# USTC-Computer-Vision/tracking

Hardware: AMD Instinct MI355X
Metric: MixtureOfGaussianV2BGS throughput (Mpixels/s; concurrent 1080p30 streams in streams_1080p30) (higher is better)
Workload: dtype f32

## Files before the change

### tracking_amd/csrc/bgs_hip.hip

```cpp
#include "../../include/bgs_hip.h"

#include <hip/hip_runtime.h>

#include <algorithm>
#include <chrono>
#include <cmath>
#include <cstdarg>
#include <cstdio>
#include <cstdlib>
#include <cstring>
#include <mutex>
#include <new>
#include <string>
#include <atomic>
#include <vector>

#include "kernel_gmg.h"
#include "kernel_ingest.h"
#include "kernel_kde.h"
#include "kernel_dp2.h"
#include "kernel_lb.h"
#include "kernel_cc.h"
#include "kernel_dp.h"
#include "kernel_mog1.h"
// ... 294 lines not shown
  static const bool debug = getenv("BGS_DEBUG_STAT") != nullptr;
  if (debug)
    fprintf(stderr, "[bgs] mog2 auto: %u record slots sampled, %.3f live, %.3f needed after the summaries -> mode %d (now %d)\n", total, lf, nf, want, e->mog2_sparse_now);
  if (want != e->mog2_sparse_now && (clear || want == e->mog2_sparse_want)) e->mog2_sparse_now = want;
  e->mog2_sparse_want = want;
}
void mog2_stat_post(bgs_engine* e, hipStream_t s) {
  const int i = (int)(e->stat_seq % bgs_engine::kStatSlots);
  (void)hipMemcpyAsync(e->h_stat + 3 * i, e->d_stat, 3 * sizeof(unsigned), hipMemcpyDeviceToHost, s);
  (void)hipMemsetAsync(e->d_stat, 0, 3 * sizeof(unsigned), s);
  (void)hipEventRecord(e->stat_ev[i], s);
  e->stat_posted[i] = true;
  e->stat_seq++;
}

int launch_mog2(bgs_engine* e, bgs::Mog2Args& a, hipStream_t s, bool timed = true) {
  const bgs_params& p = e->p;
  a.shadow = p.mog2_detect_shadows && (!p.enable_threshold || ((p.mog2_shadow_value > p.threshold) != (255 > p.threshold)));
  a.want_bg = a.bgimg != nullptr, a.packed = a.fg_bits != nullptr;
  a.xcd_swizzle = e->xcd_swizzle, a.complete = e->mog2_complete;
  const bool autom = timed && e->mog2_sparse == 3;
  if (autom) mog2_stat_read(e);
  int mode = e->mog2_sparse == 3 ? e->mog2_sparse_now : e->mog2_sparse;
  if (mode >= 4 && (a.shadow || a.want_bg)) mode = 2;
  if (autom && mode != 4) {
    const unsigned n = e->mog2_launches++;
    if ((n & (n < 64 ? 3u : 15u)) == 0) mode = 4;
  }
  a.sparse = mode;
  a.stat = (autom && mode == 4) ? e->d_stat : nullptr;
  if (a.packed && a.npix % 64) return fail(BGS_ERR_UNSUPPORTED, "packed mask needs pixels %% 64 == 0");
  Timed t(e, s, "mog2_update_kernel", timed);
  const dim3 grid(blocks_for(a.npix)), block(bgs::kBlock);
  unsigned every = 1;
  while (grid.x / every > 256) every <<= 1;
  a.stat_mask = every - 1;
  static const unsigned lds_pad = getenv("BGS_MOG2_LDS_PAD") ? (unsigned)std::max(0, std::min(65536, atoi(getenv("BGS_MOG2_LDS_PAD")))) : 0u;
  if (mode >= 4)
    hipLaunchKernelGGL((bgs::mog2_update_kernel<bgs::kMog2Filter>), grid, block, lds_pad, s, a);
  else if (mode >= 2)
    hipLaunchKernelGGL((bgs::mog2_update_kernel<bgs::kMog2Count>), grid, block, lds_pad, s, a);
  else
    hipLaunchKernelGGL((bgs::mog2_update_kernel<bgs::kMog2Eager>), grid, block, lds_pad, s, a);
  if (a.stat) mog2_stat_post(e, s);
  return BGS_OK;
}

void mog1_fill_args(const bgs_engine* e, bgs::Mog1Args& m, double lr) {
  const bgs_params& p = e->p;
  const int C = e->ch;
  const double defaultNoiseSigma = 30 * 0.5;
  m.alpha = (float)lr, m.T = (float)p.mog1_background_ratio, m.vT = (float)p.mog1_var_threshold;
  m.w0 = (float)0.05;
  m.sk0 = C == 3 ? (float)(m.w0 / (defaultNoiseSigma * 2 * std::sqrt(3.))) : (float)(m.w0 / (defaultNoiseSigma * 2));
  m.var0 = (float)(defaultNoiseSigma * defaultNoiseSigma * 4);
  m.minVar = (float)(p.mog1_noise_sigma * p.mog1_noise_sigma);
  m.thr = p.threshold, m.enable_thr = p.enable_threshold, m.packed = m.fg_bits != nullptr, m.xcd_swizzle = e->xcd_swizzle;
}

void mog2_fill_args(const bgs_engine* e, bgs::Mog2Args& m, double lr) {
  const bgs_params& p = e->p;
  m.state = e->mog2_state;
  m.alphaT = (float)lr, m.alpha1 = 1.f - m.alphaT, m.prune = (float)(-lr * (double)p.mog2_ct);
  m.Tb = p.mog2_var_threshold, m.TB = p.mog2_background_ratio, m.Tg = p.mog2_var_threshold_gen;
  m.varInit = p.mog2_var_init, m.varMin = p.mog2_var_min, m.varMax = p.mog2_var_max, m.tau = p.mog2_tau;
  m.thr = p.threshold, m.enable_thr = p.enable_threshold, m.shadow_val = p.mog2_shadow_value;
}

void mog2_clear(bgs_engine* e, const bgs::Mog2Args& m, hipStream_t s) {
  hipLaunchKernelGGL(bgs::mog2_clear_kernel, dim3(blocks_for(m.npix)), dim3(bgs::kBlock), 0, s, m);
}

// ... 1355 lines not shown
  if (!strcmp(plane, "hostpath")) {
    double rec[15] = {0};
    for (size_t i = 0; i < e->pin.size(); ++i) rec[i % 3] += e->pin[i].pinned, rec[3 + i % 3] += e->pin[i].refused;
    rec[6] = (double)e->diag_reg_calls, rec[7] = e->diag_reg_ms, rec[8] = (double)e->diag_unreg_calls, rec[9] = (double)e->diag_frames;
    rec[10] = (double)e->diag_h2d_bytes, rec[11] = (double)e->diag_d2h_bytes, rec[12] = e->diag_stage_in_ms, rec[13] = e->diag_stage_out_ms, rec[14] = (double)e->arenas.size();
    if (cap < sizeof(rec)) return fail(BGS_ERR_STATE, "buffer too small for plane %s", plane);
    memcpy(dst, rec, sizeof(rec));
    return (int64_t)sizeof(rec);
  }
  if (!strcmp(plane, "placement")) {
    float rec[2] = {e->vmm.base ? (float)(e->vmm.chunk >> 20) : 0.f, (float)e->vmm.handles.size()};
    if (cap < sizeof(rec)) return fail(BGS_ERR_STATE, "buffer too small for plane %s", plane);
    memcpy(dst, rec, sizeof(rec));
    return (int64_t)sizeof(rec);
  }
  if (e->algo == BGS_MOG2) {
    int p0 = -1, np = 0;
    if (!strcmp(plane, "w")) p0 = 0, np = 5;
    if (!strcmp(plane, "var")) p0 = 5, np = 5;
    if (!strcmp(plane, "mu")) p0 = 10, np = 15;
    if (!strcmp(plane, "summary")) p0 = 100, np = 5;
    const bool nm = !strcmp(plane, "nmodes") || !strcmp(plane, "summary_valid");
    const bool want_valid = !strcmp(plane, "summary_valid");
    if (p0 >= 0 || nm) {
      const size_t need = nm ? n : (size_t)np * n * 4;
      if (cap < need) return fail(BGS_ERR_STATE, "buffer too small for plane %s", plane);
      const size_t T = bgs::kMog2Tile, TB = bgs::kMog2TileBytes;
      const size_t t0 = off / T, t1 = (off + n + T - 1) / T;
      std::vector<uint8_t> tiles((t1 - t0) * TB);
      if (d2h_staged(tiles.data(), e->mog2_state + t0 * TB, tiles.size()) != BGS_OK) return fail(BGS_ERR_HIP, "hipMemcpy failed");
      for (size_t i = 0; i < n; ++i) {
        const size_t sp = off + i, in = sp % T;
        const uint8_t* tb = tiles.data() + (sp / T - t0) * TB;
        const float* w = reinterpret_cast<const float*>(tb) + in;
        const float* rec = reinterpret_cast<const float*>(tb + bgs::kMog2RecOff) + in * 4;
        const uint16_t* sum = reinterpret_cast<const uint16_t*>(tb + bgs::kMog2SumOff) + in;
        const unsigned meta = reinterpret_cast<const uint16_t*>(tb + bgs::kMog2MetaOff)[in];
        if (nm) {
          ((uint8_t*)dst)[i] = want_valid ? (uint8_t)((meta >> 15) & 1u) : (uint8_t)bgs::mog2_meta_count(meta);
          continue;
        }
        for (int r = 0; r < bgs::kMog2K; ++r) {
          const unsigned f = (meta >> (3 * r)) & 7u;
          const float* rc = f ? rec + (size_t)(f - 1) * T * 4 : nullptr;
          if (p0 == 100) ((uint32_t*)dst)[(size_t)r * n + i] = f ? sum[(size_t)(f - 1) * T] : 0u;
          if (p0 == 0) ((float*)dst)[(size_t)r * n + i] = f ? w[(size_t)r * T] : 0.f;
          if (p0 == 5) ((float*)dst)[(size_t)r * n + i] = f ? rc[0] : 0.f;
          if (p0 == 10)
            for (int c = 0; c < 3; ++c) ((float*)dst)[((size_t)r * 3 + c) * n + i] = f ? rc[1 + c] : 0.f;
        }
      }
      return (int64_t)need;
    }
  }
  if ((e->algo == BGS_SUBSENSE || e->algo == BGS_LOBSTER) && e->ss) return ss_get_state(e, stream, plane, dst, cap);
  if (e->algo == BGS_KDE && e->kde_samples) return kde_get_state(e, stream, plane, dst, cap);
  if (is_lb(e->algo) && e->lb_model) return lb_get_state(e, stream, plane, dst, cap);
  if ((e->algo == BGS_DP_PRATI_MEDIOD && e->pm_samples) || (e->algo == BGS_DP_TEXTURE && e->tex_r)) return dp2_get_state(e, stream, plane, dst, cap);
  if (is_dp(e->algo)) {
    const int planes = dp_planes_of(e);
    const char* fname = (e->algo == BGS_DP_WREN_GA) ? "gauss" : (e->algo == BGS_DP_MEAN) ? "mean" : "modes";
    if (planes && !strcmp(plane, fname)) return dp_export_planes(e, stream, planes, dst, cap);
    if (e->state_ch == 1 && !strcmp(plane, "nmodes")) return copy_bytes(e->bgstate + off, n);
    if (e->state_ch == 3 && !strcmp(plane, "median")) return copy_bytes(e->bgstate + off * 3, n * 3);
    return fail(BGS_ERR_STATE, "unknown state plane '%s' for algorithm %d", plane, (int)e->algo);
  }
  if (e->algo == BGS_GMG && e->gmg_rec) {
    const size_t F = (size_t)e->p.gmg_max_features;
    std::vector<uint8_t> nf(n);
    if (d2h_staged(nf.data(), e->gmg_nfeat + off, n) != BGS_OK) return fail(BGS_ERR_HIP, "hipMemcpy failed");
    if (!strcmp(plane, "nfeatures")) {
      if (cap < n * 4) return fail(BGS_ERR_STATE, "buffer too small for plane %s", plane);
      for (size_t i = 0; i < n; ++i) ((int32_t*)dst)[i] = nf[i];
      return (int64_t)(n * 4);
    }
    if (!strcmp(plane, "colors") || !strcmp(plane, "weights")) {
      if (cap < n * F * 4) return fail(BGS_ERR_STATE, "buffer too small for plane %s", plane);
      const int which = !strcmp(plane, "colors") ? 0 : 1;
      std::vector<uint32_t> recs(n * 2);
// ... 564 lines not shown
```

### tracking_amd/csrc/kernel_mog2.h

```cpp
#pragma once
#include "bgs_device.h"

namespace bgs {

constexpr int kMog2K = 5;
#ifndef BGS_MOG2_TILE
#define BGS_MOG2_TILE 256
#endif
constexpr int kMog2Tile = BGS_MOG2_TILE;
constexpr size_t kMog2TileBytes = (size_t)kMog2Tile * (4 * kMog2K + 2 * kMog2K + 16 * kMog2K + 2);
constexpr size_t kMog2SumOff = (size_t)kMog2Tile * 4 * kMog2K;
constexpr size_t kMog2RecOff = kMog2SumOff + (size_t)kMog2Tile * 2 * kMog2K;
constexpr size_t kMog2MetaOff = kMog2RecOff + (size_t)kMog2Tile * 16 * kMog2K;
static_assert(kMog2Tile % 64 == 0, "a wave never straddles two tiles");

struct Mog2Args {
  const uint8_t* frame;
  uint8_t* fg;
  uint8_t* bgimg;
  uint64_t* fg_bits;
  uint8_t* state;
  size_t state_off;
  size_t npix;
  float alphaT, alpha1, prune;
  float Tb, TB, Tg, varInit, varMin, varMax, tau;
  int thr, enable_thr, shadow_val;
  int shadow, want_bg, packed;
  unsigned* stat;
  unsigned stat_mask;
  int sparse;
  int complete;
  int xcd_swizzle;
};

struct Mog2Ptr {
  float* w;
  uint16_t* sum;
  float4* rec;
  uint16_t* meta;
};
__device__ __forceinline__ Mog2Ptr mog2_ptr(uint8_t* state, size_t sp) {
  uint8_t* tb = state + (sp / kMog2Tile) * kMog2TileBytes;
  const size_t in = sp % kMog2Tile;
  Mog2Ptr p;
  p.w = reinterpret_cast<float*>(tb) + in;
  p.sum = reinterpret_cast<uint16_t*>(tb + kMog2SumOff) + in;
  p.rec = reinterpret_cast<float4*>(tb + kMog2RecOff) + in;
  p.meta = reinterpret_cast<uint16_t*>(tb + kMog2MetaOff) + in;
  return p;
}
__device__ __host__ __forceinline__ int mog2_meta_count(unsigned meta) {
  unsigned t = (meta | (meta >> 1) | (meta >> 2)) & 0x1249u;
  t = (t & 1u) + ((t >> 3) & 1u) + ((t >> 6) & 1u) + ((t >> 9) & 1u) + ((t >> 12) & 1u);
  return (int)t;
}

constexpr float kMog2SumVar = 32.f, kMog2SumVarTight = 24.f;
__device__ __host__ __forceinline__ uint32_t mog2_summary(float var, float m0, float m1, float m2) {
  const bool inside = m0 >= 0.f && m0 < 256.f && m1 >= 0.f && m1 < 256.f && m2 >= 0.f && m2 < 256.f;
  const uint32_t cls = (inside && var <= kMog2SumVarTight) ? 0u : 1u;
  const uint32_t q0 = inside ? (uint32_t)(int)m0 >> 3 : 0u, q1 = inside ? (uint32_t)(int)m1 >> 3 : 0u, q2 = inside ? (uint32_t)(int)m2 >> 3 : 0u;
  return q0 | (q1 << 5) | (q2 << 10) | (cls << 15);
}
__device__ __host__ __forceinline__ bool mog2_summary_ok(uint32_t word, float var, float m0, float m1, float m2) {
  const float b0 = (float)((word & 0x1fu) << 3), b1 = (float)(((word >> 5) & 0x1fu) << 3), b2 = (float)(((word >> 10) & 0x1fu) << 3);
  const float e0 = m0 - b0, e1 = m1 - b1, e2 = m2 - b2;
  const bool means = (e0 >= -2.f && e0 <= 9.f) && (e1 >= -2.f && e1 <= 9.f) && (e2 >= -2.f && e2 <= 9.f);
  const bool tightable = var <= kMog2SumVarTight && m0 >= 0.f && m0 < 256.f && m1 >= 0.f && m1 < 256.f && m2 >= 0.f && m2 < 256.f;
  return (word >> 15) ? !tightable : (means && var <= kMog2SumVar);
}
__device__ __host__ __forceinline__ uint32_t mog2_tq(float Tmax) {
  const float c = 3.f * kMog2SumVar * Tmax;
  return c < 1.0e9f ? (uint32_t)(int)c + 4u : 0xffffffffu;
}
__device__ __forceinline__ uint32_t mog2_pixq(uint32_t pix) { return (pix >> 3) & 0x1f1f1fu; }
__device__ __forceinline__ bool mog2_reject(uint32_t word, uint32_t pixq, uint32_t tq) {
  const uint32_t qb = (word & 0x1fu) | ((word & 0x3e0u) << 3) | ((word & 0x7c00u) << 6);
  const uint32_t S = __builtin_amdgcn_sad_u8(pixq, qb, 0u);
  const uint32_t B = 8u * S - 28u;
  return S > 3u && !(word >> 15) && B * B > tq;
}

// ... 142 lines not shown
  nmodes = nNewModes;
  if (!fitsPDF) {
    const int slot = (nmodes == kMog2K) ? s.sl[kMog2K - 1] : nmodes + 1;
    const int mode = (nmodes == kMog2K) ? kMog2K - 1 : nmodes++;
#pragma unroll
    for (int k = 0; k < kMog2K; ++k) {
      if (k == mode) {
        s.w[k] = (nmodes == 1) ? 1.f : alphaT;
        s.sl[k] = slot;
        if constexpr (ORD == kMog2Ranked) R.rc[k] = make_float4(a.varInit, x0, x1, x2);
      } else if (nmodes != 1 && k < nmodes - 1) {
        s.w[k] *= alpha1;
      }
    }
    out = make_float4(a.varInit, x0, x1, x2);
    hit = slot;
    bool moving = true;
#pragma unroll
    for (int i = kMog2K - 1; i > 0; --i) {
      if (i <= nmodes - 1) {
        moving = moving && !(alphaT < s.w[i - 1]);
        if (moving) mog2_swap<ORD>(s, R, i, i - 1);
      }
    }
  }
  nmodes_io = nmodes;
  if (background) return 0;
  if (a.shadow) {
    if (mog2_shadow<ORD>(s, R, hit, out, nmodes, x0, x1, x2, a)) return a.shadow_val;
  }
  return 255;
}

template <int ORD>
__device__ __forceinline__ int mog2_pixel_lockstep(Mog2Px& s, const Mog2Recs& R, const int ncand, const int wave_cand, int& nmodes_io, float x0, float x1, float x2,
                                                   const Mog2Args& a, int& hit, float4& out, const float alphaT, const float alpha1, const float prune) {
  static_assert(ORD == kMog2Compact || ORD == kMog2BySlot, "records by slot or compacted");
  bool background = false, fitsPDF = false;
  int nmodes = nmodes_io;
  const int nNewModes = nmodes;
  float totalWeight = 0.f;
  hit = 0;
  out = make_float4(0.f, 0.f, 0.f, 0.f);
  unsigned cm = 0, bgm = 0, mm = 0;
#pragma unroll
  for (int j = 0; j < kMog2K; ++j) {
    if (j < wave_cand) {
      const float4 v = R.rc[j];
      const float d0 = v.y - x0, d1 = v.z - x1, d2 = v.w - x2;
      const float dist2 = d0 * d0 + d1 * d1 + d2 * d2;
      const int code = ORD == kMog2BySlot ? j + 1 : R.kj[j] + 1;
      const bool is = j < ncand;
      cm |= (unsigned)is << code;
      bgm |= (unsigned)(is && dist2 < a.Tb * v.x) << code;
      mm |= (unsigned)(is && dist2 < a.Tg * v.x) << code;
    }
  }
  float wmatch = 0.f;
  int rstar = 0;
#pragma unroll
  for (int mode = 0; mode < kMog2K; ++mode) {
    if (mode < nmodes) {
      float weight = alpha1 * s.w[mode] + prune;
      const int code = s.sl[mode];
      if (!fitsPDF && ((cm >> code) & 1u)) {
        if (totalWeight < a.TB && ((bgm >> code) & 1u)) background = true;
        if ((mm >> code) & 1u) {
// ... 29 lines not shown
    }
  }
  totalWeight = div_rn(1.f, totalWeight);
#pragma unroll
  for (int mode = 0; mode < kMog2K; ++mode)
    if (mode < nmodes) s.w[mode] *= totalWeight;
  nmodes = nNewModes;
  if (!fitsPDF) {
    const int slot = (nmodes == kMog2K) ? s.sl[kMog2K - 1] : nmodes + 1;
    const int mode = (nmodes == kMog2K) ? kMog2K - 1 : nmodes++;
#pragma unroll
    for (int k = 0; k < kMog2K; ++k) {
      if (k == mode) {
        s.w[k] = (nmodes == 1) ? 1.f : alphaT;
        s.sl[k] = slot;
      } else if (nmodes != 1 && k < nmodes - 1) {
        s.w[k] *= alpha1;
      }
    }
    out = make_float4(a.varInit, x0, x1, x2);
    hit = slot;
    bool moving = true;
    Mog2Recs none;
#pragma unroll
    for (int i = kMog2K - 1; i > 0; --i) {
      if (i <= nmodes - 1) {
        moving = moving && !(alphaT < s.w[i - 1]);
        if (moving) mog2_swap<ORD>(s, none, i, i - 1);
      }
    }
  }
  nmodes_io = nmodes;
  if (background) return 0;
  if (a.shadow) {
    if (mog2_shadow<ORD>(s, R, hit, out, nmodes, x0, x1, x2, a)) return a.shadow_val;
  }
  return 255;
}

template <int ORD>
__device__ __forceinline__ void mog2_background(const Mog2Px& s, const Mog2Recs& R, int hit, float4 out, int nmodes, float TB, int& b0, int& b1, int& b2) {
  float v0 = 0.f, v1 = 0.f, v2 = 0.f, totalWeight = 0.f;
  bool stop = false;
#pragma unroll
  for (int g = 0; g < kMog2K; ++g) {
    if (g < nmodes && !stop) {
      const float4 v = mog2_rec_now<ORD>(s, R, g, hit, out);
      const float w = s.w[g];
      v0 += w * v.y;
      v1 += w * v.z;
      v2 += w * v.w;
      totalWeight += w;
      if (totalWeight > TB) stop = true;
    }
  }
  const float inv = div_rn(1.f, totalWeight);
  b0 = sat_u8(v0 * inv), b1 = sat_u8(v1 * inv), b2 = sat_u8(v2 * inv);
}

__device__ __forceinline__ void mog2_group_or(unsigned v, unsigned& or2, unsigned& or8, unsigned& or16) {
  v |= (unsigned)__builtin_amdgcn_mov_dpp((int)v, 0xB1, 0xf, 0xf, true);
  or2 = v;
  v |= (unsigned)__builtin_amdgcn_mov_dpp((int)v, 0x4E, 0xf, 0xf, true);
  v |= (unsigned)__builtin_amdgcn_mov_dpp((int)v, 0x141, 0xf, 0xf, true);
  or8 = v;
  v |= (unsigned)__builtin_amdgcn_mov_dpp((int)v, 0x140, 0xf, 0xf, true);
  or16 = v;
}

constexpr int kMog2ClipMax = 8;
struct Mog2ClipArgs {
  Mog2Args m;
  size_t frame_stride;
  size_t fg_stride, bg_stride, bits_stride;
  float alphaT[kMog2ClipMax], alpha1[kMog2ClipMax], prune[kMog2ClipMax];
};

enum { kMog2Eager = 1, kMog2Count = 2, kMog2Filter = 4 };

template <int MODE, int T>
__device__ __forceinline__ void mog2_body(const Mog2Args& a, const size_t frame_stride, const size_t fg_stride, const size_t bg_stride, const size_t bits_stride,
                                          const float* alphaT, const float* alpha1, const float* prune) {
  static_assert(T == 1 || MODE == kMog2Eager, "clip launches load eagerly");
  constexpr int ORD = MODE == kMog2Filter ? kMog2Compact : T > 1 ? kMog2Ranked : kMog2BySlot;
  size_t blk = blockIdx.x;
  if (a.xcd_swizzle) {
    const size_t per = gridDim.x >> 3, main = per << 3;
    if (blk < main) blk = (blk & 7) * per + (blk >> 3);
  }
  const size_t p0 = blk * kBlock + threadIdx.x;
  if (p0 >= a.npix) return;
  const size_t sp = a.state_off + p0;
  uint32_t pix[T];
#pragma unroll
  for (int t = 0; t < T; ++t) {
    const uint8_t* f = a.frame + (size_t)t * frame_stride + p0 * 3;
    pix[t] = (uint32_t)f[0] | ((uint32_t)f[1] << 8) | ((uint32_t)f[2] << 16);
  }
  const Mog2Ptr mp = mog2_ptr(a.state, sp);
  const unsigned meta_raw = *mp.meta;
  const unsigned meta_in = meta_raw & 0x7fffu;
  const bool valid_in = (meta_raw >> 15) & 1u;
  const int nm_in = mog2_meta_count(meta_in);
  const bool dense = MODE == kMog2Eager && a.sparse == 0;
  const bool can_reject = !a.shadow && !a.want_bg;
  float wv[kMog2K];
  uint32_t sm[kMog2K];
  Mog2Recs R;
  R.cnt = kMog2K;
  unsigned rej = 0;
  int wave_cand = kMog2K;
#pragma unroll
  for (int k = 0; k < kMog2K; ++k) R.kj[k] = k, sm[k] = 0u;
  if constexpr (MODE == kMog2Eager) {
#pragma unroll
    for (int k = 0; k < kMog2K; ++k) {
      wv[k] = mp.w[(size_t)k * kMog2Tile];
      R.rc[k] = mp.rec[(size_t)k * kMog2Tile];
      if (dense) sm[k] = mp.sum[(size_t)k * kMog2Tile];
    }
  } else if constexpr (MODE == kMog2Count) {
    wv[0] = mp.w[0];
    R.rc[0] = mp.rec[0];
    int wave_nm = 0;
#pragma unroll
    for (int n = 1; n <= kMog2K; ++n)
      if (__any(nm_in >= n)) wave_nm = n;
    wave_cand = wave_nm <= 2 ? 2 : wave_nm;
    if (wave_nm <= 2) {
      const size_t idx = (size_t)(1 < nm_in ? 1 : 0) * kMog2Tile;
      wv[1] = mp.w[idx], R.rc[1] = mp.rec[idx];
#pragma unroll
      for (int k = 2; k < kMog2K; ++k) wv[k] = 0.f, R.rc[k] = make_float4(0.f, 0.f, 0.f, 0.f);
    } else {
#pragma unroll
      for (int k = 1; k < kMog2K; ++k) {
        const size_t idx = (size_t)(k < nm_in ? k : 0) * kMog2Tile;
        wv[k] = mp.w[idx], R.rc[k] = mp.rec[idx];
      }
    }
#pragma unroll
    for (int k = 0; k < kMog2K; ++k) wv[k] = k < nm_in ? wv[k] : 0.f;
    R.cnt = nm_in;
  } else {
#pragma unroll
    for (int k = 0; k < kMog2K; ++k) wv[k] = mp.w[(size_t)k * kMog2Tile], sm[k] = mp.sum[(size_t)k * kMog2Tile];
    const uint32_t tq = mog2_tq(a.Tb > a.Tg ? a.Tb : a.Tg), pixq = mog2_pixq(pix[0]);
    unsigned need = 0;
#pragma unroll
    for (int k = 0; k < kMog2K; ++k) {
      const bool live = k < nm_in;
      wv[k] = live ? wv[k] : 0.f;
      sm[k] = live ? sm[k] : 0u;
      const bool r = live && valid_in && can_reject && mog2_reject(sm[k], pixq, tq);
      rej |= (unsigned)r << (k + 1);
      need |= (unsigned)(live && !r) << k;
    }
    R.cnt = __popc(need);
    const int k_first = need ? __ffs(need) - 1 : 0;
    R.kj[0] = k_first;
    if (!__any(R.cnt > 1)) {
      wave_cand = 1;
      R.rc[0] = mp.rec[(size_t)k_first * kMog2Tile];
#pragma unroll
      for (int j = 1; j < kMog2K; ++j) R.rc[j] = make_float4(0.f, 0.f, 0.f, 0.f), R.kj[j] = k_first;
    } else {
      unsigned left = need & (need - 1);
#pragma unroll
      for (int j = 1; j < kMog2K; ++j) {
        R.kj[j] = left ? __ffs(left) - 1 : k_first;
        left &= left - 1;
      }
#pragma unroll
      for (int j = 0; j < kMog2K; ++j) R.rc[j] = mp.rec[(size_t)R.kj[j] * kMog2Tile];
    }
    if (a.stat && (blockIdx.x & a.stat_mask) == 0) {
      int would = R.cnt;
      if (!valid_in && can_reject) {
        would = 0;
#pragma unroll
        for (int j = 0; j < kMog2K; ++j) {
          const float4 c = R.rc[j];
          if (j < R.cnt && !mog2_reject(mog2_summary(c.x, c.y, c.z, c.w), pixq, tq)) ++would;
        }
      }
      unsigned s_live = 0, s_need = 0;
#pragma unroll
      for (int bit = 0; bit < 3; ++bit) {
        s_live += (unsigned)__popcll(__ballot((nm_in >> bit) & 1)) << bit;
        s_need += (unsigned)__popcll(__ballot((would >> bit) & 1)) << bit;
      }
      const unsigned lanes = (unsigned)__popcll(__ballot(1));
      if ((threadIdx.x & (kWave - 1)) == 0) {
        atomicAdd(a.stat, lanes * kMog2K);
        atomicAdd(a.stat + 1, s_live);
        atomicAdd(a.stat + 2, s_need);
      }
    }
  }
  Mog2Px s;
#pragma unroll
  for (int r = 0; r < kMog2K; ++r) s.sl[r] = (int)((meta_in >> (3 * r)) & 7u), s.w[r] = wv[r];
  if constexpr (ORD == kMog2Ranked) {
    Mog2Recs Q;
#pragma unroll
    for (int r = 0; r < kMog2K; ++r) Q.rc[r] = mog2_pick<true>(R, s.sl[r]);
#pragma unroll
    for (int r = 0; r < kMog2K; ++r) R.rc[r] = Q.rc[r];
  }
  unsigned dirty = 0;
  int nm = nm_in, hit = 0;
  float4 out = make_float4(0.f, 0.f, 0.f, 0.f);
#pragma unroll
  for (int t = 0; t < T; ++t) {
    const float x0 = (float)(pix[t] & 0xffu), x1 = (float)((pix[t] >> 8) & 0xffu), x2 = (float)(pix[t] >> 16);
    int raw;
    if constexpr (ORD == kMog2Ranked)
      raw = mog2_pixel<ORD>(s, R, nm, x0, x1, x2, a, hit, out, alphaT[t], alpha1[t], prune[t], rej);
    else
      raw = mog2_pixel_lockstep<ORD>(s, R, R.cnt, wave_cand, nm, x0, x1, x2, a, hit, out, alphaT[t], alpha1[t], prune[t]);
    const int m = thr_bin(raw, a.thr, a.enable_thr);
    if (a.fg) a.fg[(size_t)t * fg_stride + p0] = (uint8_t)m;
    if (a.packed) store_packed_mask<1>(a.fg_bits + (size_t)t * bits_stride, p0, (uint32_t)(m != 0), true);
    if (a.want_bg) {
      int b0, b1, b2;
      mog2_background<ORD>(s, R, hit, out, nm, a.TB, b0, b1, b2);
      uint8_t* o = a.bgimg + (size_t)t * bg_stride + p0 * 3;
      o[0] = (uint8_t)b0, o[1] = (uint8_t)b1, o[2] = (uint8_t)b2;
    }
    dirty |= 1u << hit;
  }
  unsigned d = 0;
#pragma unroll
  for (int r = 0; r < kMog2K; ++r) d |= (unsigned)(s.w[r] != wv[r]) << r;
  d |= (dirty >> 1) << 6;
  bool valid_out = false;
  if constexpr (MODE == kMog2Filter) {
    uint32_t old = 0;
#pragma unroll
    for (int q = 0; q < kMog2K; ++q) old = hit == q + 1 ? sm[q] : old;
    const bool keep = valid_in && hit <= nm_in && mog2_summary_ok(old, out.x, out.y, out.z, out.w);
    if (__any(!keep)) {
#pragma unroll
      for (int q = 0; q < kMog2K; ++q) {
        const bool changed = hit == q + 1;
        if ((changed && !keep) || (!valid_in && q < nm)) {
          const float4 v = mog2_pick_now<false>(R, q + 1, hit, out);
          sm[q] = mog2_summary(v.x, v.y, v.z, v.w);
          d |= 1u << (11 + q);
        }
      }
    }
    valid_out = true;
  }
  unsigned meta_out = valid_out ? 0x8000u : 0u;
#pragma unroll
  for (int r = 0; r < kMog2K; ++r) meta_out |= (unsigned)s.sl[r] << (3 * r);
  d |= (unsigned)(meta_out != meta_raw) << 5;
  if (dense) {
    d = 0xffffu;
  } else if (a.complete) {
    unsigned d2, d8, d16;
    mog2_group_or(d, d2, d8, d16);
    unsigned c = (d8 & 0x1fu) | (d16 & 0x20u);
    if constexpr (MODE == kMog2Filter) c |= d16 & 0xf800u;
    if constexpr (MODE == kMog2Eager) c |= d2 & 0x7c0u;
    d |= c;
  }
#pragma unroll
  for (int r = 0; r < kMog2K; ++r)
    if ((d >> r) & 1u) mp.w[(size_t)r * kMog2Tile] = s.w[r];
  if ((d >> 5) & 1u) *mp.meta = (uint16_t)meta_out;
  if constexpr (MODE == kMog2Eager) {
#pragma unroll
    for (int q = 0; q < kMog2K; ++q) {
      if ((d >> (11 + q)) & 1u) mp.sum[(size_t)q * kMog2Tile] = (uint16_t)sm[q];
      if ((d >> (6 + q)) & 1u) {
        float4 v;
        if constexpr (T == 1) {
          const bool h = hit == q + 1;
          v = make_float4(h ? out.x : R.rc[q].x, h ? out.y : R.rc[q].y, h ? out.z : R.rc[q].z, h ? out.w : R.rc[q].w);
        } else {
          v = make_float4(0.f, 0.f, 0.f, 0.f);
#pragma unroll
          for (int r = 0; r < kMog2K; ++r) {
            const bool h = s.sl[r] == q + 1;
            v.x = h ? R.rc[r].x : v.x, v.y = h ? R.rc[r].y : v.y, v.z = h ? R.rc[r].z : v.z, v.w = h ? R.rc[r].w : v.w;
          }
        }
        mp.rec[(size_t)q * kMog2Tile] = v;
      }
    }
  } else {
    mp.rec[(size_t)(hit - 1) * kMog2Tile] = out;
    if constexpr (MODE == kMog2Filter) {
#pragma unroll
      for (int q = 0; q < kMog2K; ++q)
        if ((d >> (11 + q)) & 1u) mp.sum[(size_t)q * kMog2Tile] = (uint16_t)sm[q];
    }
  }
}

template <int MODE>
__global__ __launch_bounds__(kBlock) void mog2_update_kernel(const Mog2Args a) {
  mog2_body<MODE, 1>(a, 0, 0, 0, 0, &a.alphaT, &a.alpha1, &a.prune);
}

template <int T>
__global__ __launch_bounds__(kBlock) void mog2_clip_kernel(const Mog2ClipArgs c) {
  mog2_body<kMog2Eager, T>(c.m, c.frame_stride, c.fg_stride, c.bg_stride, c.bits_stride, c.alphaT, c.alpha1, c.prune);
}

__global__ __launch_bounds__(kBlock) void mog2_clear_kernel(const Mog2Args a) {
  const size_t p = (size_t)blockIdx.x * kBlock + threadIdx.x;
  if (p >= a.npix) return;
  const Mog2Ptr mp = mog2_ptr(a.state, a.state_off + p);
#pragma unroll
  for (int k = 0; k < kMog2K; ++k) {
    mp.w[(size_t)k * kMog2Tile] = 0.f;
    mp.sum[(size_t)k * kMog2Tile] = 0;
    mp.rec[(size_t)k * kMog2Tile] = make_float4(0.f, 0.f, 0.f, 0.f);
  }
  *mp.meta = 0;
}

}
```

Measured before the change: 65520.

## Split MoG2 weights into high and low 16-bit planes with independent dirty writes

Stores each float mixture weight as two separate 16-bit planes (high half and low half) inside the tile, and tracks dirtiness for each half separately. Only the halves that changed are written back, which cuts write traffic when only low mantissa bits change or only the high half changes. The wave-level OR now uses the 16-lane group for weight dirtiness instead of the 8-lane group. In exchange, every weight read becomes two narrow loads plus a combine, there is more bookkeeping in the dirty mask, and the state export path has to reassemble the halves.

```diff
diff --git a/tracking_amd/csrc/bgs_hip.hip b/tracking_amd/csrc/bgs_hip.hip
--- a/tracking_amd/csrc/bgs_hip.hip
+++ b/tracking_amd/csrc/bgs_hip.hip
@@ -1777,7 +1777,8 @@
       for (size_t i = 0; i < n; ++i) {
         const size_t sp = off + i, in = sp % T;
         const uint8_t* tb = tiles.data() + (sp / T - t0) * TB;
-        const float* w = reinterpret_cast<const float*>(tb) + in;
+        const uint16_t* whi = reinterpret_cast<const uint16_t*>(tb) + in;
+        const uint16_t* wlo = reinterpret_cast<const uint16_t*>(tb + bgs::kMog2WloOff) + in;
         const float* rec = reinterpret_cast<const float*>(tb + bgs::kMog2RecOff) + in * 4;
         const uint16_t* sum = reinterpret_cast<const uint16_t*>(tb + bgs::kMog2SumOff) + in;
         const unsigned meta = reinterpret_cast<const uint16_t*>(tb + bgs::kMog2MetaOff)[in];
@@ -1789,7 +1790,7 @@
           const unsigned f = (meta >> (3 * r)) & 7u;
           const float* rc = f ? rec + (size_t)(f - 1) * T * 4 : nullptr;
           if (p0 == 100) ((uint32_t*)dst)[(size_t)r * n + i] = f ? sum[(size_t)(f - 1) * T] : 0u;
-          if (p0 == 0) ((float*)dst)[(size_t)r * n + i] = f ? w[(size_t)r * T] : 0.f;
+          if (p0 == 0) ((uint32_t*)dst)[(size_t)r * n + i] = f ? ((uint32_t)whi[(size_t)r * T] << 16) | wlo[(size_t)r * T] : 0u;
           if (p0 == 5) ((float*)dst)[(size_t)r * n + i] = f ? rc[0] : 0.f;
           if (p0 == 10)
             for (int c = 0; c < 3; ++c) ((float*)dst)[((size_t)r * 3 + c) * n + i] = f ? rc[1 + c] : 0.f;
diff --git a/tracking_amd/csrc/kernel_mog2.h b/tracking_amd/csrc/kernel_mog2.h
--- a/tracking_amd/csrc/kernel_mog2.h
+++ b/tracking_amd/csrc/kernel_mog2.h
@@ -9,6 +9,7 @@
 #endif
 constexpr int kMog2Tile = BGS_MOG2_TILE;
 constexpr size_t kMog2TileBytes = (size_t)kMog2Tile * (4 * kMog2K + 2 * kMog2K + 16 * kMog2K + 2);
+constexpr size_t kMog2WloOff = (size_t)kMog2Tile * 2 * kMog2K;
 constexpr size_t kMog2SumOff = (size_t)kMog2Tile * 4 * kMog2K;
 constexpr size_t kMog2RecOff = kMog2SumOff + (size_t)kMog2Tile * 2 * kMog2K;
 constexpr size_t kMog2MetaOff = kMog2RecOff + (size_t)kMog2Tile * 16 * kMog2K;
@@ -34,7 +35,8 @@
 };
 
 struct Mog2Ptr {
-  float* w;
+  uint16_t* whi;
+  uint16_t* wlo;
   uint16_t* sum;
   float4* rec;
   uint16_t* meta;
@@ -43,11 +45,15 @@
   uint8_t* tb = state + (sp / kMog2Tile) * kMog2TileBytes;
   const size_t in = sp % kMog2Tile;
   Mog2Ptr p;
-  p.w = reinterpret_cast<float*>(tb) + in;
+  p.whi = reinterpret_cast<uint16_t*>(tb) + in;
+  p.wlo = reinterpret_cast<uint16_t*>(tb + kMog2WloOff) + in;
   p.sum = reinterpret_cast<uint16_t*>(tb + kMog2SumOff) + in;
   p.rec = reinterpret_cast<float4*>(tb + kMog2RecOff) + in;
   p.meta = reinterpret_cast<uint16_t*>(tb + kMog2MetaOff) + in;
   return p;
+}
+__device__ __forceinline__ float mog2_load_w(const Mog2Ptr& p, size_t idx) {
+  return __uint_as_float(((uint32_t)p.whi[idx] << 16) | (uint32_t)p.wlo[idx]);
 }
 __device__ __host__ __forceinline__ int mog2_meta_count(unsigned meta) {
   unsigned t = (meta | (meta >> 1) | (meta >> 2)) & 0x1249u;
@@ -378,12 +384,11 @@
   b0 = sat_u8(v0 * inv), b1 = sat_u8(v1 * inv), b2 = sat_u8(v2 * inv);
 }
 
-__device__ __forceinline__ void mog2_group_or(unsigned v, unsigned& or2, unsigned& or8, unsigned& or16) {
+__device__ __forceinline__ void mog2_group_or(unsigned v, unsigned& or2, unsigned& or16) {
   v |= (unsigned)__builtin_amdgcn_mov_dpp((int)v, 0xB1, 0xf, 0xf, true);
   or2 = v;
   v |= (unsigned)__builtin_amdgcn_mov_dpp((int)v, 0x4E, 0xf, 0xf, true);
   v |= (unsigned)__builtin_amdgcn_mov_dpp((int)v, 0x141, 0xf, 0xf, true);
-  or8 = v;
   v |= (unsigned)__builtin_amdgcn_mov_dpp((int)v, 0x140, 0xf, 0xf, true);
   or16 = v;
 }
@@ -435,12 +440,12 @@
   if constexpr (MODE == kMog2Eager) {
 #pragma unroll
     for (int k = 0; k < kMog2K; ++k) {
-      wv[k] = mp.w[(size_t)k * kMog2Tile];
+      wv[k] = mog2_load_w(mp, (size_t)k * kMog2Tile);
       R.rc[k] = mp.rec[(size_t)k * kMog2Tile];
       if (dense) sm[k] = mp.sum[(size_t)k * kMog2Tile];
     }
   } else if constexpr (MODE == kMog2Count) {
-    wv[0] = mp.w[0];
+    wv[0] = mog2_load_w(mp, 0);
     R.rc[0] = mp.rec[0];
     int wave_nm = 0;
 #pragma unroll
@@ -449,14 +454,14 @@
     wave_cand = wave_nm <= 2 ? 2 : wave_nm;
     if (wave_nm <= 2) {
       const size_t idx = (size_t)(1 < nm_in ? 1 : 0) * kMog2Tile;
-      wv[1] = mp.w[idx], R.rc[1] = mp.rec[idx];
+      wv[1] = mog2_load_w(mp, idx), R.rc[1] = mp.rec[idx];
 #pragma unroll
       for (int k = 2; k < kMog2K; ++k) wv[k] = 0.f, R.rc[k] = make_float4(0.f, 0.f, 0.f, 0.f);
     } else {
 #pragma unroll
       for (int k = 1; k < kMog2K; ++k) {
         const size_t idx = (size_t)(k < nm_in ? k : 0) * kMog2Tile;
-        wv[k] = mp.w[idx], R.rc[k] = mp.rec[idx];
+        wv[k] = mog2_load_w(mp, idx), R.rc[k] = mp.rec[idx];
       }
     }
 #pragma unroll
@@ -464,7 +469,7 @@
     R.cnt = nm_in;
   } else {
 #pragma unroll
-    for (int k = 0; k < kMog2K; ++k) wv[k] = mp.w[(size_t)k * kMog2Tile], sm[k] = mp.sum[(size_t)k * kMog2Tile];
+    for (int k = 0; k < kMog2K; ++k) wv[k] = mog2_load_w(mp, (size_t)k * kMog2Tile), sm[k] = mp.sum[(size_t)k * kMog2Tile];
     const uint32_t tq = mog2_tq(a.Tb > a.Tg ? a.Tb : a.Tg), pixq = mog2_pixq(pix[0]);
     unsigned need = 0;
 #pragma unroll
@@ -552,7 +557,11 @@
   }
   unsigned d = 0;
 #pragma unroll
-  for (int r = 0; r < kMog2K; ++r) d |= (unsigned)(s.w[r] != wv[r]) << r;
+  for (int r = 0; r < kMog2K; ++r) {
+    const uint32_t x = __float_as_uint(s.w[r]) ^ __float_as_uint(wv[r]);
+    d |= (unsigned)((x >> 16) != 0u) << r;
+    d |= (unsigned)((x & 0xffffu) != 0u) << (16 + r);
+  }
   d |= (dirty >> 1) << 6;
   bool valid_out = false;
   if constexpr (MODE == kMog2Filter) {
@@ -578,18 +587,21 @@
   for (int r = 0; r < kMog2K; ++r) meta_out |= (unsigned)s.sl[r] << (3 * r);
   d |= (unsigned)(meta_out != meta_raw) << 5;
   if (dense) {
-    d = 0xffffu;
+    d = 0x1fffffu;
   } else if (a.complete) {
-    unsigned d2, d8, d16;
-    mog2_group_or(d, d2, d8, d16);
-    unsigned c = (d8 & 0x1fu) | (d16 & 0x20u);
+    unsigned d2, d16;
+    mog2_group_or(d, d2, d16);
+    unsigned c = d16 & 0x1f003fu;
     if constexpr (MODE == kMog2Filter) c |= d16 & 0xf800u;
     if constexpr (MODE == kMog2Eager) c |= d2 & 0x7c0u;
     d |= c;
   }
 #pragma unroll
-  for (int r = 0; r < kMog2K; ++r)
-    if ((d >> r) & 1u) mp.w[(size_t)r * kMog2Tile] = s.w[r];
+  for (int r = 0; r < kMog2K; ++r) {
+    const uint32_t wb = __float_as_uint(s.w[r]);
+    if ((d >> r) & 1u) mp.whi[(size_t)r * kMog2Tile] = (uint16_t)(wb >> 16);
+    if ((d >> (16 + r)) & 1u) mp.wlo[(size_t)r * kMog2Tile] = (uint16_t)wb;
+  }
   if ((d >> 5) & 1u) *mp.meta = (uint16_t)meta_out;
   if constexpr (MODE == kMog2Eager) {
 #pragma unroll
@@ -637,7 +649,8 @@
   const Mog2Ptr mp = mog2_ptr(a.state, a.state_off + p);
 #pragma unroll
   for (int k = 0; k < kMog2K; ++k) {
-    mp.w[(size_t)k * kMog2Tile] = 0.f;
+    mp.whi[(size_t)k * kMog2Tile] = 0;
+    mp.wlo[(size_t)k * kMog2Tile] = 0;
     mp.sum[(size_t)k * kMog2Tile] = 0;
     mp.rec[(size_t)k * kMog2Tile] = make_float4(0.f, 0.f, 0.f, 0.f);
   }
```

Result: slower. 63410 (-3.2%).

## Split MOG2 filter mode into a multi-tile walk kernel with prefetched headers

Applied to the files above, without the earlier changes.

Moves the sparse filter path of the MOG2 update into a dedicated kernel where each block walks several consecutive 256-pixel runs. While it computes one run, it software-prefetches the next run's pixel, meta, weight and summary headers. It also moves the meta row ahead of the record planes so the header sits in one contiguous aligned block. Shadow and background extras are compiled out of this path, and tile addressing is computed once per wave when state_off is 64-aligned. The trade-off is fewer, longer-lived blocks, more register pressure (with a waves_per_eu hint), and a changed state layout that must stay consistent across all kernels.

```diff
diff --git a/tracking_amd/csrc/bgs_hip.hip b/tracking_amd/csrc/bgs_hip.hip
--- a/tracking_amd/csrc/bgs_hip.hip
+++ b/tracking_amd/csrc/bgs_hip.hip
@@ -350,12 +350,15 @@
   if (a.packed && a.npix % 64) return fail(BGS_ERR_UNSUPPORTED, "packed mask needs pixels %% 64 == 0");
   Timed t(e, s, "mog2_update_kernel", timed);
   const dim3 grid(blocks_for(a.npix)), block(bgs::kBlock);
+  const dim3 walk((grid.x + bgs::kMog2Walk - 1) / bgs::kMog2Walk);
   unsigned every = 1;
   while (grid.x / every > 256) every <<= 1;
   a.stat_mask = every - 1;
   static const unsigned lds_pad = getenv("BGS_MOG2_LDS_PAD") ? (unsigned)std::max(0, std::min(65536, atoi(getenv("BGS_MOG2_LDS_PAD")))) : 0u;
-  if (mode >= 4)
-    hipLaunchKernelGGL((bgs::mog2_update_kernel<bgs::kMog2Filter>), grid, block, lds_pad, s, a);
+  if (mode >= 4 && a.state_off % 64 == 0)
+    hipLaunchKernelGGL(bgs::mog2_update_walk_kernel<true>, walk, block, lds_pad, s, a);
+  else if (mode >= 4)
+    hipLaunchKernelGGL(bgs::mog2_update_walk_kernel<false>, walk, block, lds_pad, s, a);
   else if (mode >= 2)
     hipLaunchKernelGGL((bgs::mog2_update_kernel<bgs::kMog2Count>), grid, block, lds_pad, s, a);
   else
diff --git a/tracking_amd/csrc/kernel_mog2.h b/tracking_amd/csrc/kernel_mog2.h
--- a/tracking_amd/csrc/kernel_mog2.h
+++ b/tracking_amd/csrc/kernel_mog2.h
@@ -10,8 +10,12 @@
 constexpr int kMog2Tile = BGS_MOG2_TILE;
 constexpr size_t kMog2TileBytes = (size_t)kMog2Tile * (4 * kMog2K + 2 * kMog2K + 16 * kMog2K + 2);
 constexpr size_t kMog2SumOff = (size_t)kMog2Tile * 4 * kMog2K;
-constexpr size_t kMog2RecOff = kMog2SumOff + (size_t)kMog2Tile * 2 * kMog2K;
-constexpr size_t kMog2MetaOff = kMog2RecOff + (size_t)kMog2Tile * 16 * kMog2K;
+constexpr size_t kMog2MetaOff = kMog2SumOff + (size_t)kMog2Tile * 2 * kMog2K;
+constexpr size_t kMog2RecOff = kMog2MetaOff + (size_t)kMog2Tile * 2;
+static_assert(kMog2RecOff + (size_t)kMog2Tile * 16 * kMog2K == kMog2TileBytes, "the four parts fill the tile");
+static_assert(kMog2RecOff == (size_t)kMog2Tile * 32 && (kMog2Tile != 256 || kMog2RecOff == 8192), "header block: 8 KiB of a 256-pixel tile");
+static_assert(kMog2Tile % 256 != 0 || (kMog2RecOff % 4096 == 0 && (kMog2Tile * 16) % 4096 == 0 && kMog2TileBytes % 4096 == 0), "every record plane is a run of aligned 4 KiB blocks");
+static_assert(kMog2MetaOff % 16 == 0, "meta row 16-byte aligned");
 static_assert(kMog2Tile % 64 == 0, "a wave never straddles two tiles");
 
 struct Mog2Args {
@@ -256,7 +260,7 @@
   return 255;
 }
 
-template <int ORD>
+template <int ORD, bool EXTRAS = true>
 __device__ __forceinline__ int mog2_pixel_lockstep(Mog2Px& s, const Mog2Recs& R, const int ncand, const int wave_cand, int& nmodes_io, float x0, float x1, float x2,
                                                    const Mog2Args& a, int& hit, float4& out, const float alphaT, const float alpha1, const float prune) {
   static_assert(ORD == kMog2Compact || ORD == kMog2BySlot, "records by slot or compacted");
@@ -352,8 +356,10 @@
   }
   nmodes_io = nmodes;
   if (background) return 0;
-  if (a.shadow) {
-    if (mog2_shadow<ORD>(s, R, hit, out, nmodes, x0, x1, x2, a)) return a.shadow_val;
+  if constexpr (EXTRAS) {
+    if (a.shadow) {
+      if (mog2_shadow<ORD>(s, R, hit, out, nmodes, x0, x1, x2, a)) return a.shadow_val;
+    }
   }
   return 255;
 }
@@ -401,8 +407,8 @@
 template <int MODE, int T>
 __device__ __forceinline__ void mog2_body(const Mog2Args& a, const size_t frame_stride, const size_t fg_stride, const size_t bg_stride, const size_t bits_stride,
                                           const float* alphaT, const float* alpha1, const float* prune) {
-  static_assert(T == 1 || MODE == kMog2Eager, "clip launches load eagerly");
-  constexpr int ORD = MODE == kMog2Filter ? kMog2Compact : T > 1 ? kMog2Ranked : kMog2BySlot;
+  static_assert(MODE == kMog2Eager || (MODE == kMog2Count && T == 1), "clip launches load eagerly; the filter kernel is mog2_filter_walk");
+  constexpr int ORD = T > 1 ? kMog2Ranked : kMog2BySlot;
   size_t blk = blockIdx.x;
   if (a.xcd_swizzle) {
     const size_t per = gridDim.x >> 3, main = per << 3;
@@ -420,15 +426,13 @@
   const Mog2Ptr mp = mog2_ptr(a.state, sp);
   const unsigned meta_raw = *mp.meta;
   const unsigned meta_in = meta_raw & 0x7fffu;
-  const bool valid_in = (meta_raw >> 15) & 1u;
   const int nm_in = mog2_meta_count(meta_in);
   const bool dense = MODE == kMog2Eager && a.sparse == 0;
-  const bool can_reject = !a.shadow && !a.want_bg;
   float wv[kMog2K];
   uint32_t sm[kMog2K];
   Mog2Recs R;
   R.cnt = kMog2K;
-  unsigned rej = 0;
+  const unsigned rej = 0;
   int wave_cand = kMog2K;
 #pragma unroll
   for (int k = 0; k < kMog2K; ++k) R.kj[k] = k, sm[k] = 0u;
@@ -439,7 +443,7 @@
       R.rc[k] = mp.rec[(size_t)k * kMog2Tile];
       if (dense) sm[k] = mp.sum[(size_t)k * kMog2Tile];
     }
-  } else if constexpr (MODE == kMog2Count) {
+  } else {
     wv[0] = mp.w[0];
     R.rc[0] = mp.rec[0];
     int wave_nm = 0;
@@ -462,61 +466,6 @@
 #pragma unroll
     for (int k = 0; k < kMog2K; ++k) wv[k] = k < nm_in ? wv[k] : 0.f;
     R.cnt = nm_in;
-  } else {
-#pragma unroll
-    for (int k = 0; k < kMog2K; ++k) wv[k] = mp.w[(size_t)k * kMog2Tile], sm[k] = mp.sum[(size_t)k * kMog2Tile];
-    const uint32_t tq = mog2_tq(a.Tb > a.Tg ? a.Tb : a.Tg), pixq = mog2_pixq(pix[0]);
-    unsigned need = 0;
-#pragma unroll
-    for (int k = 0; k < kMog2K; ++k) {
-      const bool live = k < nm_in;
-      wv[k] = live ? wv[k] : 0.f;
-      sm[k] = live ? sm[k] : 0u;
-      const bool r = live && valid_in && can_reject && mog2_reject(sm[k], pixq, tq);
-      rej |= (unsigned)r << (k + 1);
-      need |= (unsigned)(live && !r) << k;
-    }
-    R.cnt = __popc(need);
-    const int k_first = need ? __ffs(need) - 1 : 0;
-    R.kj[0] = k_first;
-    if (!__any(R.cnt > 1)) {
-      wave_cand = 1;
-      R.rc[0] = mp.rec[(size_t)k_first * kMog2Tile];
-#pragma unroll
-      for (int j = 1; j < kMog2K; ++j) R.rc[j] = make_float4(0.f, 0.f, 0.f, 0.f), R.kj[j] = k_first;
-    } else {
-      unsigned left = need & (need - 1);
-#pragma unroll
-      for (int j = 1; j < kMog2K; ++j) {
-        R.kj[j] = left ? __ffs(left) - 1 : k_first;
-        left &= left - 1;
-      }
-#pragma unroll
-      for (int j = 0; j < kMog2K; ++j) R.rc[j] = mp.rec[(size_t)R.kj[j] * kMog2Tile];
-    }
-    if (a.stat && (blockIdx.x & a.stat_mask) == 0) {
-      int would = R.cnt;
-      if (!valid_in && can_reject) {
-        would = 0;
-#pragma unroll
-        for (int j = 0; j < kMog2K; ++j) {
-          const float4 c = R.rc[j];
-          if (j < R.cnt && !mog2_reject(mog2_summary(c.x, c.y, c.z, c.w), pixq, tq)) ++would;
-        }
-      }
-      unsigned s_live = 0, s_need = 0;
-#pragma unroll
-      for (int bit = 0; bit < 3; ++bit) {
-        s_live += (unsigned)__popcll(__ballot((nm_in >> bit) & 1)) << bit;
-        s_need += (unsigned)__popcll(__ballot((would >> bit) & 1)) << bit;
-      }
-      const unsigned lanes = (unsigned)__popcll(__ballot(1));
-      if ((threadIdx.x & (kWave - 1)) == 0) {
-        atomicAdd(a.stat, lanes * kMog2K);
-        atomicAdd(a.stat + 1, s_live);
-        atomicAdd(a.stat + 2, s_need);
-      }
-    }
   }
   Mog2Px s;
 #pragma unroll
@@ -554,26 +503,7 @@
 #pragma unroll
   for (int r = 0; r < kMog2K; ++r) d |= (unsigned)(s.w[r] != wv[r]) << r;
   d |= (dirty >> 1) << 6;
-  bool valid_out = false;
-  if constexpr (MODE == kMog2Filter) {
-    uint32_t old = 0;
-#pragma unroll
-    for (int q = 0; q < kMog2K; ++q) old = hit == q + 1 ? sm[q] : old;
-    const bool keep = valid_in && hit <= nm_in && mog2_summary_ok(old, out.x, out.y, out.z, out.w);
-    if (__any(!keep)) {
-#pragma unroll
-      for (int q = 0; q < kMog2K; ++q) {
-        const bool changed = hit == q + 1;
-        if ((changed && !keep) || (!valid_in && q < nm)) {
-          const float4 v = mog2_pick_now<false>(R, q + 1, hit, out);
-          sm[q] = mog2_summary(v.x, v.y, v.z, v.w);
-          d |= 1u << (11 + q);
-        }
-      }
-    }
-    valid_out = true;
-  }
-  unsigned meta_out = valid_out ? 0x8000u : 0u;
+  unsigned meta_out = 0;
 #pragma unroll
   for (int r = 0; r < kMog2K; ++r) meta_out |= (unsigned)s.sl[r] << (3 * r);
   d |= (unsigned)(meta_out != meta_raw) << 5;
@@ -583,7 +513,6 @@
     unsigned d2, d8, d16;
     mog2_group_or(d, d2, d8, d16);
     unsigned c = (d8 & 0x1fu) | (d16 & 0x20u);
-    if constexpr (MODE == kMog2Filter) c |= d16 & 0xf800u;
     if constexpr (MODE == kMog2Eager) c |= d2 & 0x7c0u;
     d |= c;
   }
@@ -613,17 +542,209 @@
     }
   } else {
     mp.rec[(size_t)(hit - 1) * kMog2Tile] = out;
-    if constexpr (MODE == kMog2Filter) {
-#pragma unroll
-      for (int q = 0; q < kMog2K; ++q)
-        if ((d >> (11 + q)) & 1u) mp.sum[(size_t)q * kMog2Tile] = (uint16_t)sm[q];
-    }
+  }
+}
+
+#ifndef BGS_MOG2_WALK
+#define BGS_MOG2_WALK 4
+#endif
+constexpr int kMog2Walk = BGS_MOG2_WALK;
+
+struct Mog2Head {
+  uint32_t px01, px2;
+  unsigned meta;
+  float w[kMog2K];
+  uint32_t sm[kMog2K];
+};
+struct Mog2Lane {
+  size_t first;
+  uint32_t off;
+  bool active;
+  Mog2Ptr mp;
+};
+template <bool UNI>
+__device__ __forceinline__ Mog2Lane mog2_lane(const Mog2Args& a, const size_t c) {
+  Mog2Lane L;
+  L.first = c * kBlock;
+  const size_t left = a.npix - L.first;
+  const uint32_t last = left < (size_t)kBlock ? (uint32_t)left - 1u : (uint32_t)kBlock - 1u;
+  L.active = threadIdx.x <= last;
+  L.off = L.active ? threadIdx.x : last;
+  const size_t s0 = a.state_off + L.first;
+  if constexpr (UNI) {
+    const size_t tile = (s0 + (uint32_t)__builtin_amdgcn_readfirstlane((int)L.off)) / kMog2Tile;
+    uint8_t* tb = a.state + tile * kMog2TileBytes;
+    const uint32_t in = ((uint32_t)s0 + L.off) % (uint32_t)kMog2Tile;
+    L.mp.w = reinterpret_cast<float*>(tb) + in;
+    L.mp.sum = reinterpret_cast<uint16_t*>(tb + kMog2SumOff) + in;
+    L.mp.rec = reinterpret_cast<float4*>(tb + kMog2RecOff) + in;
+    L.mp.meta = reinterpret_cast<uint16_t*>(tb + kMog2MetaOff) + in;
+  } else {
+    L.mp = mog2_ptr(a.state, s0 + L.off);
+  }
+  return L;
+}
+__device__ __forceinline__ void mog2_head_load(const Mog2Args& a, const Mog2Lane& L, Mog2Head& h) {
+  const uint8_t* f = a.frame + L.first * 3 + L.off * 3u;
+  uint16_t lo;
+  __builtin_memcpy(&lo, f, 2);
+  h.px01 = lo, h.px2 = f[2];
+  h.meta = *L.mp.meta;
+#pragma unroll
+  for (int k = 0; k < kMog2K; ++k) h.w[k] = L.mp.w[(size_t)k * kMog2Tile], h.sm[k] = L.mp.sum[(size_t)k * kMog2Tile];
+}
+
+template <bool UNI>
+__device__ __forceinline__ void mog2_filter_walk(const Mog2Args& a) {
+  constexpr int ORD = kMog2Compact;
+  size_t blk = blockIdx.x;
+  if (a.xcd_swizzle) {
+    const size_t per = gridDim.x >> 3, main = per << 3;
+    if (blk < main) blk = (blk & 7) * per + (blk >> 3);
+  }
+  const size_t runs = (a.npix + kBlock - 1) / kBlock, c0 = blk * kMog2Walk;
+  if (c0 >= runs) return;
+  const int ntile = (int)(runs - c0 < (size_t)kMog2Walk ? runs - c0 : (size_t)kMog2Walk);
+  const uint32_t tq = mog2_tq(a.Tb > a.Tg ? a.Tb : a.Tg);
+  const float alphaT = a.alphaT, alpha1 = a.alpha1, prune = a.prune;
+  Mog2Head h;
+  mog2_head_load(a, mog2_lane<UNI>(a, c0), h);
+#pragma unroll 1
+  for (int i = 0; i < ntile; ++i) {
+    const size_t c = c0 + i;
+#ifdef BGS_MOG2_PRIO
+    __builtin_amdgcn_s_setprio(2);
+#endif
+    const Mog2Lane L = mog2_lane<UNI>(a, c);
+    const Mog2Ptr mp = L.mp;
+    asm volatile("" : "+v"(h.px01), "+v"(h.px2), "+v"(h.meta));
+    const uint32_t pix = h.px01 | (h.px2 << 16);
+    const unsigned meta_raw = h.meta;
+    const unsigned meta_in = meta_raw & 0x7fffu;
+    const bool valid_in = (meta_raw >> 15) & 1u;
+    const int nm_in = mog2_meta_count(meta_in);
+    float wv[kMog2K];
+    uint32_t sm[kMog2K];
+    Mog2Recs R;
+    const uint32_t pixq = mog2_pixq(pix);
+    unsigned need = 0;
+#pragma unroll
+    for (int k = 0; k < kMog2K; ++k) {
+      const bool live = k < nm_in;
+      wv[k] = live ? h.w[k] : 0.f;
+      sm[k] = live ? h.sm[k] : 0u;
+      const bool r = live && valid_in && mog2_reject(sm[k], pixq, tq);
+      need |= (unsigned)(live && !r) << k;
+    }
+    R.cnt = __popc(need);
+    const int k_first = need ? __ffs(need) - 1 : 0;
+    R.kj[0] = k_first;
+    int wave_cand = kMog2K;
+    if (!__any(R.cnt > 1)) {
+      wave_cand = 1;
+      R.rc[0] = mp.rec[(size_t)k_first * kMog2Tile];
+#pragma unroll
+      for (int j = 1; j < kMog2K; ++j) R.rc[j] = make_float4(0.f, 0.f, 0.f, 0.f), R.kj[j] = k_first;
+    } else {
+      unsigned left = need & (need - 1);
+#pragma unroll
+      for (int j = 1; j < kMog2K; ++j) {
+        R.kj[j] = left ? __ffs(left) - 1 : k_first;
+        left &= left - 1;
+      }
+#pragma unroll
+      for (int j = 0; j < kMog2K; ++j) R.rc[j] = mp.rec[(size_t)R.kj[j] * kMog2Tile];
+    }
+    __builtin_amdgcn_sched_barrier(0);
+    Mog2Head hn;
+    mog2_head_load(a, mog2_lane<UNI>(a, i + 1 < ntile ? c + 1 : c), hn);
+#ifdef BGS_MOG2_PRIO
+    __builtin_amdgcn_s_setprio(0);
+#endif
+    if (a.stat && (c & a.stat_mask) == 0) {
+      int would = R.cnt;
+      if (!valid_in) {
+        would = 0;
+#pragma unroll
+        for (int j = 0; j < kMog2K; ++j) {
+          const float4 v = R.rc[j];
+          if (j < R.cnt && !mog2_reject(mog2_summary(v.x, v.y, v.z, v.w), pixq, tq)) ++would;
+        }
+      }
+      unsigned s_live = 0, s_need = 0;
+#pragma unroll
+      for (int bit = 0; bit < 3; ++bit) {
+        s_live += (unsigned)__popcll(__ballot(L.active && ((nm_in >> bit) & 1))) << bit;
+        s_need += (unsigned)__popcll(__ballot(L.active && ((would >> bit) & 1))) << bit;
+      }
+      const unsigned lanes = (unsigned)__popcll(__ballot(L.active));
+      if ((threadIdx.x & (kWave - 1)) == 0 && lanes) {
+        atomicAdd(a.stat, lanes * kMog2K);
+        atomicAdd(a.stat + 1, s_live);
+        atomicAdd(a.stat + 2, s_need);
+      }
+    }
+    Mog2Px s;
+#pragma unroll
+    for (int r = 0; r < kMog2K; ++r) s.sl[r] = (int)((meta_in >> (3 * r)) & 7u), s.w[r] = wv[r];
+    int nm = nm_in, hit = 0;
+    float4 out = make_float4(0.f, 0.f, 0.f, 0.f);
+    const float x0 = (float)(pix & 0xffu), x1 = (float)((pix >> 8) & 0xffu), x2 = (float)(pix >> 16);
+    const int raw = mog2_pixel_lockstep<ORD, false>(s, R, R.cnt, wave_cand, nm, x0, x1, x2, a, hit, out, alphaT, alpha1, prune);
+    const int m = thr_bin(raw, a.thr, a.enable_thr);
+#ifdef BGS_MOG2_PRIO
+    __builtin_amdgcn_s_setprio(2);
+#endif
+    if (a.fg && L.active) (a.fg + L.first)[L.off] = (uint8_t)m;
+    if (a.packed) store_packed_mask<1>(a.fg_bits, L.first + L.off, (uint32_t)(m != 0), L.active);
+    unsigned d = 0;
+#pragma unroll
+    for (int r = 0; r < kMog2K; ++r) d |= (unsigned)(s.w[r] != wv[r]) << r;
+    uint32_t old = 0;
+#pragma unroll
+    for (int q = 0; q < kMog2K; ++q) old = hit == q + 1 ? sm[q] : old;
+    const bool keep = valid_in && hit <= nm_in && mog2_summary_ok(old, out.x, out.y, out.z, out.w);
+    if (__any(!keep)) {
+#pragma unroll
+      for (int q = 0; q < kMog2K; ++q) {
+        const bool changed = hit == q + 1;
+        if ((changed && !keep) || (!valid_in && q < nm)) {
+          const float4 v = mog2_pick_now<false>(R, q + 1, hit, out);
+          sm[q] = mog2_summary(v.x, v.y, v.z, v.w);
+          d |= 1u << (11 + q);
+        }
+      }
+    }
+    unsigned meta_out = 0x8000u;
+#pragma unroll
+    for (int r = 0; r < kMog2K; ++r) meta_out |= (unsigned)s.sl[r] << (3 * r);
+    d |= (unsigned)(meta_out != meta_raw) << 5;
+    d = L.active ? d : 0u;
+    if (a.complete) {
+      unsigned d2, d8, d16;
+      mog2_group_or(d, d2, d8, d16);
+      d |= (d8 & 0x1fu) | (d16 & 0x20u) | (d16 & 0xf800u);
+      d = L.active ? d : 0u;
+    }
+#pragma unroll
+    for (int r = 0; r < kMog2K; ++r)
+      if ((d >> r) & 1u) mp.w[(size_t)r * kMog2Tile] = s.w[r];
+    if ((d >> 5) & 1u) *mp.meta = (uint16_t)meta_out;
+    if (L.active) mp.rec[(size_t)(hit - 1) * kMog2Tile] = out;
+#pragma unroll
+    for (int q = 0; q < kMog2K; ++q)
+      if ((d >> (11 + q)) & 1u) mp.sum[(size_t)q * kMog2Tile] = (uint16_t)sm[q];
+    h = hn;
   }
 }
 
 template <int MODE>
 __global__ __launch_bounds__(kBlock) void mog2_update_kernel(const Mog2Args a) {
   mog2_body<MODE, 1>(a, 0, 0, 0, 0, &a.alphaT, &a.alpha1, &a.prune);
+}
+template <bool UNI>
+__global__ __launch_bounds__(kBlock) __attribute__((amdgpu_waves_per_eu(5))) void mog2_update_walk_kernel(const Mog2Args a) {
+  mog2_filter_walk<UNI>(a);
 }
 
 template <int T>
```

Result: no change. 64480 before, 64320 after (-0.3%).
